# huggingface/distil-whisper

Measured on AMD Instinct MI355X. Metric: training audio-seconds/s (distil-large-v3 student, 30 s clips), higher is better.
Workload: dtype bf16

## Files before the change

distil_whisper_amd/csrc/attention.hip:

```cpp
#include "common.h"
#include "../../include/dwamd.h"

#define NEG_BIG (-1.0e30f)
#ifndef DW_ATTN_DEFER
#define DW_ATTN_DEFER 8
#endif
typedef __attribute__((ext_vector_type(4))) unsigned u32x4;

struct AttnP {
    const bf16* q; const bf16* k; const bf16* v; bf16* o; float* lse;
    const bf16* d_o; float* delta; bf16* dq; bf16* dk; bf16* dv;
    long ldq, ldk, ldv, ldo, lddo, lddq, lddk, lddv;
    int B, H, Lq, Lk;
    long q_rows, kv_rows;
    float* dq_colsum;
    float* dv_colsum;
    const int* q_start; const int* q_len;
    const int* kv_start; const int* kv_len;
    int kv_B;
    int plain_order;
    float defer;
    int coff;
    float scale;
};

__device__ __forceinline__ bf16x8 pack8(const f32x16& x, int s2) {
    bf16x8 r;
#pragma unroll
    for (int e = 0; e < 8; ++e) r[e] = f2bf(x[s2 * 8 + e]);
    return r;
}

__device__ __forceinline__ bf16x8 ldg8(const bf16* base, long row, long ld, int col) {
    return *(const bf16x8*)(base + row * ld + col);
}

__device__ __forceinline__ void store_t(bf16* base, long ld, long row, bool ok, int cb, int hi, const f32x16& a,
                                        float mul) {
    if (!ok) return;
#pragma unroll
    for (int g = 0; g < 4; ++g) {
        bf16x4 w;
#pragma unroll
        for (int e = 0; e < 4; ++e) w[e] = f2bf(a[g * 4 + e] * mul);
        *(bf16x4*)(base + row * ld + cb * 32 + g * 8 + hi * 4) = w;
    }
}

__device__ __forceinline__ void store_rows(bf16* base, long ld, int row0, int nrows, char* patch, int lane,
                                           const f32x16& a0, const f32x16& a1, float mul) {
    const int hi = lane >> 5, ln = lane & 31;
    char* const wr = patch + ln * 144 + hi * 8;
#pragma unroll
    for (int cb = 0; cb < 2; ++cb) {
        const f32x16& a = cb == 0 ? a0 : a1;
#pragma unroll
        for (int g = 0; g < 4; ++g) {
            bf16x4 w;
#pragma unroll
            for (int e = 0; e < 4; ++e) w[e] = f2bf(a[g * 4 + e] * mul);
            *(bf16x4*)(wr + cb * 64 + g * 16) = w;
        }
    }
    const int rr = lane >> 3, sc = lane & 7;
    u32x4 o[4];
#pragma unroll
    for (int it = 0; it < 4; ++it) o[it] = *(const u32x4*)(patch + (it * 8 + rr) * 144 + sc * 16);
    const unsigned loff = (unsigned)(rr * (int)ld + sc * 8) * 2u;
    char* const rb = (char*)(base + (long)row0 * ld);
#pragma unroll
    for (int it = 0; it < 4; ++it)
        if (row0 + it * 8 + rr < nrows) *(u32x4*)(rb + (long)it * 8 * ld * 2 + loff) = o[it];
}

__device__ __forceinline__ void colsum_t(float* colsum, bool ok, int cb, int hi, int ln, const f32x16& a, float mul) {
#pragma unroll
    for (int r = 0; r < 16; ++r) {
        float v = ok ? bf2f(f2bf(a[r] * mul)) : 0.f;
#pragma unroll
        for (int o = 1; o < 32; o <<= 1) v += __shfl_xor(v, o);
        if (ln == 0) atomicAdd(colsum + cb * 32 + (r & 3) + 8 * (r >> 2) + 4 * hi, v);
    }
}

__device__ __forceinline__ void attn_workgroup(int ntile, int H, bool plain, int& tile, int& h, int& b) {
    const int n = gridDim.x, L = blockIdx.x;
    const int xcd = L & 7, slot = L >> 3, q = n >> 3, r = n & 7;
    const int logical = plain ? L : xcd * q + min(xcd, r) + slot;
    tile = logical % ntile;
    const int bh = logical / ntile;
    h = bh % H;
    b = bh / H;
}

template <bool CAUSAL, bool VL = false>
__global__ __launch_bounds__(256, CAUSAL ? 2 : 4) void attn_fwd_kernel(const AttnP p) {
    constexpr int NW = 4;
    __shared__ __attribute__((aligned(1024))) char smem[2 * 16384];
    const int lane = threadIdx.x & 63;
    const int wave = __builtin_amdgcn_readfirstlane(threadIdx.x >> 6);
    const int hi = lane >> 5, ln = lane & 31;
    int tile, h, b;
    attn_workgroup((p.Lq + 32 * NW - 1) / (32 * NW), p.H, p.plain_order, tile, h, b);
    const int qb0 = tile * (32 * NW);
    long q_row0 = (long)b * p.q_rows, kv_row0 = (long)b * p.kv_rows;
    int Lq = p.Lq, Lk = p.Lk;
    if constexpr (VL) {
        q_row0 = p.q_start[b];
        Lq = p.q_len[b];
        if (p.kv_start) { kv_row0 = p.kv_start[b]; Lk = p.kv_len[b]; }
        else kv_row0 = (long)min(b, p.kv_B - 1) * p.kv_rows;
        if (qb0 >= Lq) return;
    }
    const int q = qb0 + wave * 32 + ln;
    const bool q_ok = q < Lq;
    const int qc = q_ok ? q : Lq - 1;
    const bf16* Q = p.q + q_row0 * p.ldq + h * 64;
    const bf16* K = p.k + kv_row0 * p.ldk + h * 64;
    const bf16* V = p.v + kv_row0 * p.ldv + h * 64;

    bf16x8 qf[4];
// ... 156 lines not shown
            const float pb = round_bf16(pv);
            const bf16x8 v8 = *(const bf16x8*)(V + (long)k * p.ldv);
#pragma unroll
            for (int e = 0; e < 8; ++e) o[e] = fmaf(pb, bf2f(v8[e]), o[e]);
        }
    }
    l = (lane & 7) == 0 ? l : 0.f;
    l = wave_sum(l);
#pragma unroll
    for (int e = 0; e < 8; ++e) {
        o[e] += __shfl_xor(o[e], 8);
        o[e] += __shfl_xor(o[e], 16);
        o[e] += __shfl_xor(o[e], 32);
    }
    if (sub == 0) {
#pragma unroll
        for (int e = 0; e < 8; ++e) part[wave * 64 + ds + e] = o[e];
    }
    if (lane == 0) redl[wave] = l;
    __syncthreads();
    if (wave == 0) {
        float acc = 0.f, lt = 0.f;
#pragma unroll
        for (int i = 0; i < NW; ++i) { acc += part[i * 64 + lane]; lt += redl[i]; }
        bf16* O = p.o + (long)b * p.q_rows * p.ldo + h * 64;
        O[lane] = f2bf(acc / lt);
        if (p.lse && lane == 0) p.lse[(long)b * p.H + h] = (mx + __log2f(lt)) * 0.6931471805599453f;
    }
}

template <bool CAUSAL>
__global__ __launch_bounds__(256, 3) void attn_bwd_dq_kernel(const AttnP p) {
    constexpr int NW = 4;
    __shared__ __attribute__((aligned(1024))) char smem[2 * 16384];
    const int lane = threadIdx.x & 63;
    const int wave = __builtin_amdgcn_readfirstlane(threadIdx.x >> 6);
    const int hi = lane >> 5, ln = lane & 31;
    int tile, h, b;
    attn_workgroup((p.Lq + 32 * NW - 1) / (32 * NW), p.H, p.plain_order, tile, h, b);
    const int qb0 = tile * (32 * NW);
    const int q = qb0 + wave * 32 + ln;
    const bool q_ok = q < p.Lq;
    const int qc = q_ok ? q : p.Lq - 1;
    const bf16* Q = p.q + (long)b * p.Lq * p.ldq + h * 64;
    const bf16* DO = p.d_o + (long)b * p.Lq * p.lddo + h * 64;
    const bf16* K = p.k + (long)b * p.Lk * p.ldk + h * 64;
    const bf16* V = p.v + (long)b * p.Lk * p.ldv + h * 64;

    bf16x8 qf[4], gf[4];
#pragma unroll
    for (int kk = 0; kk < 4; ++kk) {
        qf[kk] = ldg8(Q, qc, p.ldq, kk * 16 + hi * 8);
        gf[kk] = ldg8(DO, qc, p.lddo, kk * 16 + hi * 8);
    }
    const long sidx = ((long)b * p.H + h) * p.Lq + qc;
    const float c = p.scale * 1.4426950408889634f;
    float dsum = 0.f;
    {
        const bf16* Orow = p.o + (long)b * p.Lq * p.ldo + h * 64;
#pragma unroll
        for (int kk = 0; kk < 4; ++kk) {
            const bf16x8 o8 = ldg8(Orow, qc, p.ldo, kk * 16 + hi * 8);
#pragma unroll
            for (int e = 0; e < 8; ++e) dsum += bf2f(o8[e]) * bf2f(gf[kk][e]);
        }
        dsum = xhalf_sum(dsum);
    }
// ... 55 lines not shown
                        const int key = kt * 64 + kb * 32 + ((r + e) & 3) + 8 * ((r + e) >> 2) + 4 * hi_o;
                        pv[e] = (key < p.Lk && (!CAUSAL || key <= q_o)) ? pv[e] : 0.f;
                    }
                }
                const f32x2 d2 = {dp[r], dp[r + 1]};
                pv = pv * d2;
                s[r] = pv[0];
                s[r + 1] = pv[1];
            }
#pragma unroll
            for (int s2 = 0; s2 < 2; ++s2) {
                const bf16x8 df = pack8(s, s2);
                const int rb = kb * 32 + s2 * 16 + hi * 4;
#pragma unroll
                for (int db = 0; db < 2; ++db)
                    acc[db] = __builtin_amdgcn_mfma_f32_32x32x16_bf16(frag_tr(tK, db, rb, rb + 8, lane), df, acc[db], 0, 0, 0);
            }
        }
    }
    };
    if constexpr (CAUSAL) tiles(std::integral_constant<int, 2>{}, 0, nkt);
    else {
        const int nfull = p.Lk >> 6;
        tiles(std::integral_constant<int, 0>{}, 0, nfull);
        tiles(std::integral_constant<int, 1>{}, nfull, nkt);
    }
    bf16* DQ = p.dq + (long)b * p.Lq * p.lddq + h * 64;
    if ((p.lddq & 7) == 0 && ((uintptr_t)p.dq & 15) == 0) {
        __syncthreads();
        store_rows(DQ, p.lddq, qb0 + wave * 32, p.Lq, smem + wave * 4608, lane, acc[0], acc[1], p.scale);
    } else {
        store_t(DQ, p.lddq, q, q_ok, 0, hi, acc[0], p.scale);
        store_t(DQ, p.lddq, q, q_ok, 1, hi, acc[1], p.scale);
    }
    if (p.dq_colsum) {
        colsum_t(p.dq_colsum + ((long)b * p.H + h) * 64, q_ok, 0, hi, ln, acc[0], p.scale);
        colsum_t(p.dq_colsum + ((long)b * p.H + h) * 64, q_ok, 1, hi, ln, acc[1], p.scale);
    }
}

template <bool CAUSAL>
__global__ __launch_bounds__(256, CAUSAL ? 2 : 3) void attn_bwd_dkv_kernel(const AttnP p) {
    constexpr int NW = 4;
    constexpr int STG = 16384 + 512;
    __shared__ __attribute__((aligned(1024))) char smem[2 * 17408];
    const int lane = threadIdx.x & 63;
    const int wave = __builtin_amdgcn_readfirstlane(threadIdx.x >> 6);
    const int hi = lane >> 5, ln = lane & 31;
    int tile, h, b;
    attn_workgroup((p.Lk + 32 * NW - 1) / (32 * NW), p.H, p.plain_order, tile, h, b);
    const int kb0 = tile * (32 * NW);
    const int key = kb0 + wave * 32 + ln;
    const bool k_ok = key < p.Lk;
    const int kc = k_ok ? key : p.Lk - 1;
    const bf16* Q = p.q + (long)b * p.Lq * p.ldq + h * 64;
    const bf16* DO = p.d_o + (long)b * p.Lq * p.lddo + h * 64;
    const bf16* K = p.k + (long)b * p.Lk * p.ldk + h * 64;
    const bf16* V = p.v + (long)b * p.Lk * p.ldv + h * 64;
    const float* DEL = p.delta + ((long)b * p.H + h) * p.Lq;
    const float* LSE = DEL + (long)p.B * p.H * p.Lq;

    bf16x8 kf[4], vf[4];
#pragma unroll
    for (int kk = 0; kk < 4; ++kk) {
        kf[kk] = ldg8(K, kc, p.ldk, kk * 16 + hi * 8);
        vf[kk] = ldg8(V, kc, p.ldv, kk * 16 + hi * 8);
    }
    const float c = p.scale * 1.4426950408889634f;
    const int nqt = (p.Lq + 63) >> 6;
    int qt0 = 0;
    if (CAUSAL) qt0 = kb0 >> 6;
    f32x16 av[2], ak[2];
#pragma unroll
    for (int r = 0; r < 16; ++r) { av[0][r] = 0.f; av[1][r] = 0.f; ak[0][r] = 0.f; ak[1][r] = 0.f; }

    auto stage = [&](int qt, int buf, int lane) __attribute__((always_inline)) {
        char* base = smem + buf * 17408;
        stage_tile64<NW>(Q, p.ldq, qt * 64, p.Lq, base, wave, lane);
// ... 67 lines not shown
                s[r + 1] = pv[1];
            }
#pragma unroll
            for (int s2 = 0; s2 < 2; ++s2) {
                const bf16x8 pf = pack8(pr, s2);
                const bf16x8 df = pack8(s, s2);
                const int rb = qb * 32 + s2 * 16 + hi * 4;
#pragma unroll
                for (int db = 0; db < 2; ++db) {
                    av[db] = __builtin_amdgcn_mfma_f32_32x32x16_bf16(frag_tr(tG, db, rb, rb + 8, lane), pf, av[db], 0, 0, 0);
                    ak[db] = __builtin_amdgcn_mfma_f32_32x32x16_bf16(frag_tr(tQ, db, rb, rb + 8, lane), df, ak[db], 0, 0, 0);
                }
            }
        }
    }
    };
    if constexpr (CAUSAL) tiles(std::integral_constant<int, 2>{}, qt0, nqt);
    else {
        const int nfull = kb0 + 32 * NW - 1 >= p.Lk ? 0 : (p.Lq >> 6);
        tiles(std::integral_constant<int, 0>{}, 0, nfull);
        tiles(std::integral_constant<int, 1>{}, nfull, nqt);
    }
    bf16* DK = p.dk + (long)b * p.Lk * p.lddk + h * 64;
    bf16* DV = p.dv + (long)b * p.Lk * p.lddv + h * 64;
    if (((p.lddk | p.lddv) & 7) == 0 && (((uintptr_t)p.dk | (uintptr_t)p.dv) & 15) == 0) {
        __syncthreads();
        store_rows(DK, p.lddk, kb0 + wave * 32, p.Lk, smem + wave * 4608, lane, ak[0], ak[1], p.scale);
        store_rows(DV, p.lddv, kb0 + wave * 32, p.Lk, smem + wave * 4608, lane, av[0], av[1], 1.0f);
    } else {
        store_t(DK, p.lddk, key, k_ok, 0, hi, ak[0], p.scale);
        store_t(DK, p.lddk, key, k_ok, 1, hi, ak[1], p.scale);
        store_t(DV, p.lddv, key, k_ok, 0, hi, av[0], 1.0f);
        store_t(DV, p.lddv, key, k_ok, 1, hi, av[1], 1.0f);
    }
    if (p.dv_colsum) {
        colsum_t(p.dv_colsum + ((long)b * p.H + h) * 64, k_ok, 0, hi, ln, av[0], 1.0f);
        colsum_t(p.dv_colsum + ((long)b * p.H + h) * 64, k_ok, 1, hi, ln, av[1], 1.0f);
    }
}

int g_attn_plain_order = 0;
int g_attn_defer = DW_ATTN_DEFER;
int g_attn_decode = 1;
static int check_ld(int64_t ld) { return (ld & 7) ? DW_EINVAL : DW_OK; }

extern "C" int dw_attn_fwd_ex(const void* q, const void* k, const void* v, void* o, float* lse, int B, int H, int Lq,
                              int Lk, int64_t ldq, int64_t ldk, int64_t ldv, int64_t ldo, int64_t q_batch_rows,
                              int64_t kv_batch_rows, int causal, float scale, void* stream);

extern "C" int dw_attn_fwd(const void* q, const void* k, const void* v, void* o, float* lse, int B, int H, int Lq,
                           int Lk, int64_t ldq, int64_t ldk, int64_t ldv, int64_t ldo, int causal, float scale,
                           void* stream) {
    if (!lse) return DW_EINVAL;
    return dw_attn_fwd_ex(q, k, v, o, lse, B, H, Lq, Lk, ldq, ldk, ldv, ldo, Lq, Lk, causal, scale, stream);
}

extern "C" int dw_attn_fwd_ex(const void* q, const void* k, const void* v, void* o, float* lse, int B, int H, int Lq,
                              int Lk, int64_t ldq, int64_t ldk, int64_t ldv, int64_t ldo, int64_t q_batch_rows,
                              int64_t kv_batch_rows, int causal, float scale, void* stream) {
    DW_CLEAR_ERR();
    if (!q || !k || !v || !o || B <= 0 || H <= 0 || Lq <= 0 || Lk <= 0) return DW_EINVAL;
    if (q_batch_rows < Lq || kv_batch_rows < Lk) return DW_EINVAL;
    if ((int64_t)Lk * ldk >= (1LL << 31) || (int64_t)Lk * ldv >= (1LL << 31)) return DW_EINVAL;
    if (check_ld(ldq) || check_ld(ldk) || check_ld(ldv) || (ldo & 3)) return DW_EINVAL;
    if (((uintptr_t)q & 15) || ((uintptr_t)k & 15) || ((uintptr_t)v & 15) || ((uintptr_t)o & 7)) return DW_EINVAL;
    AttnP p = {};
    p.q = (const bf16*)q; p.k = (const bf16*)k; p.v = (const bf16*)v; p.o = (bf16*)o; p.lse = lse;
    p.ldq = ldq; p.ldk = ldk; p.ldv = ldv; p.ldo = ldo;
    p.B = B; p.H = H; p.Lq = Lq; p.Lk = Lk; p.scale = scale;
    p.q_rows = q_batch_rows; p.kv_rows = kv_batch_rows;
    if (causal != 0 && causal != 1 && causal != 2) return DW_EINVAL;
// ... 28 lines not shown
    if (check_ld(ldq) || check_ld(ldk) || check_ld(ldv) || (ldo & 7)) return DW_EINVAL;
    if (((uintptr_t)q & 15) || ((uintptr_t)k & 15) || ((uintptr_t)v & 15) || ((uintptr_t)o & 15)) return DW_EINVAL;
    const int64_t lk_max = kv_start ? max_q : Lk;
    if (lk_max * ldk >= (1LL << 31) || lk_max * ldv >= (1LL << 31)) return DW_EINVAL;
    AttnP p = {};
    p.q = (const bf16*)q; p.k = (const bf16*)k; p.v = (const bf16*)v; p.o = (bf16*)o; p.lse = nullptr;
    p.ldq = ldq; p.ldk = ldk; p.ldv = ldv; p.ldo = ldo;
    p.B = n_seq; p.H = H; p.Lq = max_q; p.Lk = kv_start ? max_q : Lk; p.scale = scale;
    p.q_rows = 0; p.kv_rows = kv_batch_rows; p.coff = 0;
    p.q_start = q_start; p.q_len = q_len; p.kv_start = kv_start; p.kv_len = kv_len; p.kv_B = kv_batches;
    p.plain_order = g_attn_plain_order;
    p.defer = (float)g_attn_defer;
    hipStream_t s = (hipStream_t)stream;
    dim3 grid(((max_q + 127) / 128) * H * n_seq), block(256);
    if (causal) hipLaunchKernelGGL((attn_fwd_kernel<true, true>), grid, block, 0, s, p);
    else hipLaunchKernelGGL((attn_fwd_kernel<false, true>), grid, block, 0, s, p);
    DW_CHECK_LAUNCH();
    return DW_OK;
}

extern "C" int dw_attn_bwd_ex(const void* q, const void* k, const void* v, const void* o, const void* d_o,
                              const float* lse, float* delta, void* dq, void* dk, void* dv, int B, int H, int Lq, int Lk,
                              int64_t ldq, int64_t ldk, int64_t ldv, int64_t ldo, int64_t lddo, int64_t lddq,
                              int64_t lddk, int64_t lddv, int causal, float scale, float* dq_colsum, float* dv_colsum,
                              void* stream);
extern "C" int dw_attn_bwd(const void* q, const void* k, const void* v, const void* o, const void* d_o,
                           const float* lse, float* delta, void* dq, void* dk, void* dv, int B, int H, int Lq, int Lk,
                           int64_t ldq, int64_t ldk, int64_t ldv, int64_t ldo, int64_t lddo, int64_t lddq,
                           int64_t lddk, int64_t lddv, int causal, float scale, void* stream) {
    return dw_attn_bwd_ex(q, k, v, o, d_o, lse, delta, dq, dk, dv, B, H, Lq, Lk, ldq, ldk, ldv, ldo, lddo, lddq, lddk, lddv,
                          causal, scale, nullptr, nullptr, stream);
}

extern "C" int dw_attn_bwd_ex(const void* q, const void* k, const void* v, const void* o, const void* d_o,
                              const float* lse, float* delta, void* dq, void* dk, void* dv, int B, int H, int Lq, int Lk,
                              int64_t ldq, int64_t ldk, int64_t ldv, int64_t ldo, int64_t lddo, int64_t lddq,
                              int64_t lddk, int64_t lddv, int causal, float scale, float* dq_colsum, float* dv_colsum,
                              void* stream) {
    DW_CLEAR_ERR();
    if (!q || !k || !v || !o || !d_o || !lse || !delta || !dq || !dk || !dv) return DW_EINVAL;
    if (B <= 0 || H <= 0 || Lq <= 0 || Lk <= 0) return DW_EINVAL;
    if (causal != 0 && causal != 1) return DW_EINVAL;
    if (check_ld(ldq) || check_ld(ldk) || check_ld(ldv) || check_ld(ldo) || check_ld(lddo)) return DW_EINVAL;
    if ((lddq & 3) || (lddk & 3) || (lddv & 3)) return DW_EINVAL;
    if ((int64_t)Lk * ldk >= (1LL << 31) || (int64_t)Lk * ldv >= (1LL << 31) || (int64_t)Lq * ldq >= (1LL << 31) ||
        (int64_t)Lq * lddo >= (1LL << 31))
        return DW_EINVAL;
    if (((uintptr_t)q & 15) || ((uintptr_t)k & 15) || ((uintptr_t)v & 15) || ((uintptr_t)o & 15) ||
        ((uintptr_t)d_o & 15) || ((uintptr_t)dq & 7) || ((uintptr_t)dk & 7) || ((uintptr_t)dv & 7))
        return DW_EINVAL;
    AttnP p = {};
    p.q = (const bf16*)q; p.k = (const bf16*)k; p.v = (const bf16*)v; p.o = (bf16*)o; p.lse = (float*)lse;
    p.d_o = (const bf16*)d_o; p.delta = delta; p.dq = (bf16*)dq; p.dk = (bf16*)dk; p.dv = (bf16*)dv;
    p.ldq = ldq; p.ldk = ldk; p.ldv = ldv; p.ldo = ldo; p.lddo = lddo; p.lddq = lddq; p.lddk = lddk; p.lddv = lddv;
    p.B = B; p.H = H; p.Lq = Lq; p.Lk = Lk; p.scale = scale;
    p.dq_colsum = dq_colsum; p.dv_colsum = dv_colsum;
    hipStream_t s = (hipStream_t)stream;
    dim3 gq(((Lq + 127) / 128) * H * B), gk(((Lk + 127) / 128) * H * B), block(256);
    p.plain_order = g_attn_plain_order;
    p.defer = (float)g_attn_defer;
    if (causal) hipLaunchKernelGGL(attn_bwd_dq_kernel<true>, gq, block, 0, s, p);
    else hipLaunchKernelGGL(attn_bwd_dq_kernel<false>, gq, block, 0, s, p);
    if (causal) hipLaunchKernelGGL(attn_bwd_dkv_kernel<true>, gk, block, 0, s, p);
    else hipLaunchKernelGGL(attn_bwd_dkv_kernel<false>, gk, block, 0, s, p);
    DW_CHECK_LAUNCH();
    return DW_OK;
}
```

distil_whisper_amd/csrc/elementwise.hip:

```cpp
#include "common.h"
#include "../../include/dwamd.h"

template <bool TBF, bool OBF>
__global__ __launch_bounds__(256) void embed_fwd_kernel(const int64_t* ids, const void* tok, const void* pos, void* out,
                                                        int T, int D, long nvec) {
    const long i = (long)blockIdx.x * 256 + threadIdx.x;
    if (i >= nvec) return;
    const int dv = D >> 2;
    const long row = i / dv;
    const int c = (int)(i - row * dv) * 4;
    const int t = (int)(row % T);
    const long id = ids[row];
    f32x4 a, b;
    if (TBF) {
        const bf16x4 x = *(const bf16x4*)((const bf16*)tok + id * D + c);
        const bf16x4 y = *(const bf16x4*)((const bf16*)pos + (long)t * D + c);
#pragma unroll
        for (int e = 0; e < 4; ++e) { a[e] = bf2f(x[e]); b[e] = bf2f(y[e]); }
    } else {
        a = *(const f32x4*)((const float*)tok + id * D + c);
        b = *(const f32x4*)((const float*)pos + (long)t * D + c);
    }
    if (OBF) {
        bf16x4 o;
// ... 345 lines not shown
}

extern "C" int dw_cast_f32_bf16(const float* x, void* y, int64_t n, void* stream) {
    DW_CLEAR_ERR();
    if (!x || !y || n <= 0 || ((uintptr_t)x & 15) || ((uintptr_t)y & 7)) return DW_EINVAL;
    hipLaunchKernelGGL(cast_f32_bf16_kernel, dim3(((n + 3) / 4 + 255) / 256), dim3(256), 0, (hipStream_t)stream, x,
                       (bf16*)y, (long)n);
    DW_CHECK_LAUNCH();
    return DW_OK;
}
extern "C" int dw_cast_bf16_f32(const void* x, float* y, int64_t n, void* stream) {
    DW_CLEAR_ERR();
    if (!x || !y || n <= 0 || ((uintptr_t)x & 7) || ((uintptr_t)y & 15)) return DW_EINVAL;
    hipLaunchKernelGGL(cast_bf16_f32_kernel, dim3(((n + 3) / 4 + 255) / 256), dim3(256), 0, (hipStream_t)stream,
                       (const bf16*)x, y, (long)n);
    DW_CHECK_LAUNCH();
    return DW_OK;
}

extern "C" int dw_colsum_bf16(const void* x, int64_t ld, int rows, int cols, float* out, int accumulate,
                              void* stream) {
    DW_CLEAR_ERR();
    if (!x || !out || rows <= 0 || cols <= 0 || (cols & 7) || (ld & 7) || ((uintptr_t)x & 15)) return DW_EINVAL;
    hipStream_t s = (hipStream_t)stream;
    if (!accumulate) hipLaunchKernelGGL(zero_f32_kernel, dim3((cols + 255) / 256), dim3(256), 0, s, out, cols);
    int ry = (rows + 15) / 16;
    if (ry > 64) ry = 64;
    hipLaunchKernelGGL(colsum_kernel, dim3((cols + 127) / 128, ry), dim3(256), 0, s, (const bf16*)x, (long)ld, rows,
                       cols, out);
    DW_CHECK_LAUNCH();
    return DW_OK;
}

extern "C" int dw_add(const void* a, int a_dtype, const void* b, int b_dtype, void* y, int y_dtype, int64_t n,
                      void* stream) {
    DW_CLEAR_ERR();
    if (!a || !b || !y || n <= 0) return DW_EINVAL;
    long nb = (n + 255) / 256;
    if (nb > 4096) nb = 4096;
    hipLaunchKernelGGL(add_kernel, dim3(nb), dim3(256), 0, (hipStream_t)stream, a, a_dtype, b, b_dtype, y, y_dtype,
                       (long)n);
    DW_CHECK_LAUNCH();
    return DW_OK;
}

extern "C" int dw_move_rows(const void* src, int64_t src_pitch_bytes, void* dst, int64_t dst_pitch_bytes,
                            const int32_t* idx, int n, int row_bytes, int scatter, void* stream) {
    DW_CLEAR_ERR();
    if (!src || !dst || !idx || n <= 0 || row_bytes <= 0 || (row_bytes & 15) || (src_pitch_bytes & 15) ||
        (dst_pitch_bytes & 15) || ((uintptr_t)src & 15) || ((uintptr_t)dst & 15))
        return DW_EINVAL;
    const int vpr = row_bytes >> 4;
    const long nv = (long)n * vpr;
    hipLaunchKernelGGL(move_rows_kernel, dim3((nv + 255) / 256), dim3(256), 0, (hipStream_t)stream, (const char*)src,
                       (long)src_pitch_bytes, (char*)dst, (long)dst_pitch_bytes, idx, n, vpr, scatter);
    DW_CHECK_LAUNCH();
    return DW_OK;
}

extern "C" int dw_selftest_tr16(int32_t* out, void* stream) {
    DW_CLEAR_ERR();
    if (!out) return DW_EINVAL;
    hipLaunchKernelGGL(selftest_tr16_kernel, dim3(1), dim3(64), 0, (hipStream_t)stream, out);
    DW_CHECK_LAUNCH();
    return DW_OK;
}
// ... 1 lines not shown
```

distil_whisper_amd/ops_hip.py:

```python
import ctypes as C
import math
import os

import torch

from .decoding import SEQUENCE_BIAS_MAX_SEQUENCES, SEQUENCE_BIAS_MAX_TOKENS

_HERE = os.path.dirname(os.path.abspath(__file__))
LIB_PATH = os.path.join(_HERE, "libdwamd.so")

DW_F32, DW_BF16 = 0, 1


class DwGemm(C.Structure):
    _fields_ = [
        ("a", C.c_void_p), ("b", C.c_void_p), ("c", C.c_void_p), ("bias", C.c_void_p), ("z_out", C.c_void_p),
        ("zgrad_in", C.c_void_p), ("r", C.c_void_p),
        ("lda", C.c_int64), ("ldb", C.c_int64), ("ldc", C.c_int64), ("ldz", C.c_int64), ("ldzg", C.c_int64),
        ("ldr", C.c_int64),
        ("m", C.c_int32), ("n", C.c_int32), ("k", C.c_int32),
        ("trans_a", C.c_int32), ("trans_b", C.c_int32), ("act", C.c_int32), ("c_dtype", C.c_int32),
        ("r_dtype", C.c_int32), ("r_row_mod", C.c_int32), ("round_res", C.c_int32), ("tile", C.c_int32),
        ("split_k", C.c_int32), ("atomic_acc", C.c_int32), ("slice_stride", C.c_int64),
        ("ln_x", C.c_void_p), ("ln_gamma", C.c_void_p), ("ln_beta", C.c_void_p), ("kv_out", C.c_void_p),
# ... 27 lines not shown
                             C.c_float, C.c_void_p], C.c_int),
    "dw_decode_attn_proj_rows": ([C.c_void_p, C.c_int, C.c_int64, C.c_void_p, C.c_void_p, C.c_float, C.c_void_p, C.c_void_p, C.c_void_p,
                                  C.c_void_p, C.c_int64, C.c_int64, C.c_void_p, C.c_void_p, C.c_int64, C.c_int, C.c_int, C.c_float,
                                  C.c_void_p, C.c_int32, C.c_void_p], C.c_int),
    "dw_decode_token_rows": ([C.POINTER(DwDecodeStep), C.c_void_p, C.c_int32, C.c_void_p], C.c_int),
    "dw_cross_kv_quant": ([C.c_void_p, C.c_int64, C.c_void_p, C.c_void_p, C.c_void_p, C.c_int, C.c_int, C.c_int, C.c_int, C.c_void_p],
                          C.c_int),
    "dw_decode_attn_proj_kv8": ([C.c_void_p, C.c_int, C.c_int64, C.c_void_p, C.c_void_p, C.c_float, C.c_void_p, C.c_void_p, C.c_void_p,
                                 C.c_void_p, C.c_void_p, C.c_int64, C.c_void_p, C.c_int64, C.c_int, C.c_int, C.c_int, C.c_float,
                                 C.c_void_p], C.c_int),
    "dw_slot_step": ([C.c_void_p, C.c_int, C.c_int, C.c_int64, C.c_void_p, C.c_void_p] + [C.c_int] * 4 + [C.c_void_p, C.c_int64] +
                     [C.c_void_p] * 7, C.c_int),
    "dw_slot_step_scores": ([C.c_void_p, C.c_int, C.c_int, C.c_int64, C.c_void_p, C.c_void_p] + [C.c_int] * 4 +
                            [C.c_void_p, C.c_int64] + [C.c_void_p] * 9 + [C.c_int, C.c_void_p], C.c_int),
    "dw_logmel": ([C.c_void_p, C.c_int, C.c_int, C.c_void_p, C.c_int, C.c_void_p, C.c_void_p, C.c_void_p, C.c_void_p,
                   C.c_void_p], C.c_int),
    "dw_gemm_bf16": ([C.POINTER(DwGemm), C.c_void_p], C.c_int),
    "dw_layernorm_fwd": ([C.c_void_p, C.c_int, C.c_void_p, C.c_void_p, C.c_void_p, C.c_void_p, C.c_void_p, C.c_int,
                          C.c_int, C.c_float, C.c_void_p], C.c_int),
    "dw_layernorm_bwd": ([C.c_void_p, C.c_void_p, C.c_int, C.c_void_p, C.c_void_p, C.c_void_p, C.c_void_p, C.c_int,
                          C.c_void_p, C.c_void_p, C.c_void_p, C.c_void_p, C.c_int, C.c_int, C.c_void_p, C.c_int64, C.c_void_p], C.c_int),
    "dw_layernorm_bwd_ws_bytes": ([C.c_int, C.c_int], C.c_int),
    "dw_reduce_slices_ld": ([C.c_void_p, C.c_int64, C.c_int64, C.c_int, C.c_void_p, C.c_int64, C.c_int, C.c_int, C.c_int, C.c_void_p], C.c_int),
    "dw_layernorm_fwd_ld": ([C.c_void_p, C.c_int, C.c_void_p, C.c_void_p, C.c_void_p, C.c_void_p, C.c_void_p, C.c_int,
                             C.c_int, C.c_float, C.c_int64, C.c_int64, C.c_void_p], C.c_int),
    "dw_layernorm_bwd_ld": ([C.c_void_p, C.c_void_p, C.c_int, C.c_void_p, C.c_void_p, C.c_void_p, C.c_void_p, C.c_int,
                             C.c_void_p, C.c_void_p, C.c_void_p, C.c_void_p, C.c_int, C.c_int] + [C.c_int64] * 4 + [C.c_void_p, C.c_int64, C.c_void_p], C.c_int),
    "dw_attn_fwd": ([C.c_void_p] * 5 + [C.c_int] * 4 + [C.c_int64] * 4 + [C.c_int, C.c_float, C.c_void_p], C.c_int),
    "dw_attn_fwd_ex": ([C.c_void_p] * 5 + [C.c_int] * 4 + [C.c_int64] * 6 + [C.c_int, C.c_float, C.c_void_p], C.c_int),
    "dw_attn_fwd_varlen": ([C.c_void_p] * 4 + [C.c_int] * 4 + [C.c_int64] * 4 + [C.c_void_p] * 4 + [C.c_int, C.c_int64, C.c_int, C.c_float,
                                                                                                           C.c_void_p], C.c_int),
    "dw_attn_bwd": ([C.c_void_p] * 10 + [C.c_int] * 4 + [C.c_int64] * 8 + [C.c_int, C.c_float, C.c_void_p], C.c_int),
    "dw_attn_bwd_ex": ([C.c_void_p] * 10 + [C.c_int] * 4 + [C.c_int64] * 8 + [C.c_int, C.c_float] + [C.c_void_p] * 3, C.c_int),
    "dw_distill_loss": ([C.c_void_p, C.c_void_p, C.c_void_p, C.c_int, C.c_int, C.c_int64, C.c_float, C.c_float,
                         C.c_float, C.c_float, C.c_void_p, C.c_void_p, C.c_void_p, C.c_void_p, C.c_void_p,
                         C.c_void_p], C.c_int),
    "dw_distill_loss_w": ([C.c_void_p, C.c_void_p, C.c_void_p, C.c_int, C.c_int, C.c_int64, C.c_float, C.c_void_p,
                           C.c_float, C.c_void_p, C.c_void_p, C.c_void_p, C.c_void_p, C.c_void_p, C.c_void_p], C.c_int),
    "dw_embed_fwd": ([C.c_void_p, C.c_void_p, C.c_void_p, C.c_int, C.c_void_p, C.c_int, C.c_int, C.c_int, C.c_int,
                      C.c_void_p], C.c_int),
    "dw_embed_bwd": ([C.c_void_p, C.c_void_p, C.c_void_p, C.c_void_p, C.c_int, C.c_int, C.c_int, C.c_void_p], C.c_int),
    "dw_im2col_mel": ([C.c_void_p, C.c_void_p, C.c_int, C.c_int, C.c_int, C.c_int, C.c_void_p], C.c_int),
    "dw_im2col_s2": ([C.c_void_p, C.c_void_p, C.c_int, C.c_int, C.c_int, C.c_void_p], C.c_int),
    "dw_col2im_s2_gelu_bwd": ([C.c_void_p, C.c_void_p, C.c_void_p, C.c_int, C.c_int, C.c_int, C.c_void_p], C.c_int),
    "dw_gelu_bwd": ([C.c_void_p, C.c_int, C.c_void_p, C.c_void_p, C.c_int64, C.c_void_p], C.c_int),
    "dw_pack_conv_weight": ([C.c_void_p, C.c_void_p, C.c_int, C.c_int, C.c_int, C.c_void_p], C.c_int),
    "dw_unpack_conv_grad": ([C.c_void_p, C.c_void_p, C.c_int, C.c_int, C.c_int, C.c_int, C.c_void_p], C.c_int),
    "dw_cast_f32_bf16": ([C.c_void_p, C.c_void_p, C.c_int64, C.c_void_p], C.c_int),
    "dw_cast_bf16_f32": ([C.c_void_p, C.c_void_p, C.c_int64, C.c_void_p], C.c_int),
    "dw_colsum_bf16": ([C.c_void_p, C.c_int64, C.c_int, C.c_int, C.c_void_p, C.c_int, C.c_void_p], C.c_int),
    "dw_add": ([C.c_void_p, C.c_int, C.c_void_p, C.c_int, C.c_void_p, C.c_int, C.c_int64, C.c_void_p], C.c_int),
    "dw_move_rows": ([C.c_void_p, C.c_int64, C.c_void_p, C.c_int64, C.c_void_p, C.c_int, C.c_int, C.c_int, C.c_void_p], C.c_int),
    "dw_sumsq_f32": ([C.c_void_p, C.c_int64, C.c_void_p, C.c_void_p, C.c_void_p], C.c_int),
    "dw_adamw": ([C.c_void_p] * 5 + [C.c_int64, C.c_void_p] + [C.c_float] * 2 + [C.c_double] * 5 + [C.c_int, C.c_void_p], C.c_int),
    "dw_adam_tick": ([C.c_void_p, C.c_void_p, C.c_void_p], C.c_int),
    "dw_adamw_dev": ([C.c_void_p] * 5 + [C.c_int64, C.c_void_p] + [C.c_float] * 2 + [C.c_void_p] + [C.c_double] * 2 +
                     [C.c_void_p], C.c_int),
    "dw_selftest_tr16": ([C.c_void_p, C.c_void_p], C.c_int),
    "dw_debug_set": ([C.c_int, C.c_int], C.c_int),
    "dw_reduce_slices": ([C.c_void_p, C.c_int64, C.c_int, C.c_void_p, C.c_int64, C.c_int, C.c_void_p], C.c_int),
    "dw_greedy_select": ([C.c_void_p, C.c_int, C.c_int, C.c_int64, C.c_void_p, C.c_void_p] + [C.c_int] * 5 +
                         [C.c_void_p, C.c_int64, C.c_int, C.c_int, C.c_int, C.c_int, C.c_void_p, C.c_void_p,
                          C.c_void_p], C.c_int),
    "dw_greedy_select_history": ([C.c_void_p, C.c_int, C.c_int, C.c_int64, C.c_void_p, C.c_void_p] + [C.c_int] * 5 +
                                 [C.c_void_p, C.c_int64, C.c_int, C.c_int, C.c_int, C.c_int, C.c_void_p, C.c_void_p,
                                  C.c_float, C.c_int, C.c_void_p], C.c_int),
# ... 375 lines not shown
                                              v.stride(0), out.stride(0), _p(q_start), _p(q_len),
                                              _p(q_start) if self_attention else None, _p(q_len) if self_attention else None,
                                              int(kv_batches), int(Lk), int(causal), float(scale), self._stream()), "attn_fwd_varlen")
        self._t1(e0, "attn_fwd", flops)
        return out

    def attn_fwd(self, q, k, v, B, H, Lq, Lk, causal, scale, out=None, kv_batch_rows=None):
        for t in (q, k, v):
            assert t.dtype == torch.bfloat16 and t.stride(1) == 1
        o = self.empty((B * Lq, H * 64), torch.bfloat16) if out is None else out
        assert o.dtype == torch.bfloat16 and o.stride(1) == 1 and o.shape == (B * Lq, H * 64)
        lse = self.empty((B, H, Lq), torch.float32)
        e0 = self._t0()
        self._chk(self.lib.dw_attn_fwd_ex(_p(q), _p(k), _p(v), _p(o), _p(lse), B, H, Lq, Lk, q.stride(0), k.stride(0),
                                          v.stride(0), o.stride(0), Lq, Lk if kv_batch_rows is None else kv_batch_rows,
                                          int(causal), float(scale), self._stream()), "attn_fwd")
        self._t1(e0, "attn_fwd", 4.0 * B * H * Lq * Lk * 64)
        return o, lse

    def attn_bwd(self, q, k, v, o, do, lse, B, H, Lq, Lk, causal, scale, dq=None, dk=None, dv=None, dq_colsum=None,
                 dv_colsum=None):
        if dq is None:
            dq = self.empty((B * Lq, H * 64), torch.bfloat16)
        if dk is None:
            dk = self.empty((B * Lk, H * 64), torch.bfloat16)
        if dv is None:
            dv = self.empty((B * Lk, H * 64), torch.bfloat16)
        delta = self.empty((2, B, H, Lq), torch.float32)
        for t in (q, k, v, o, do, dq, dk, dv):
            assert t.dtype == torch.bfloat16 and t.stride(1) == 1
        e0 = self._t0()
        for t in (dq_colsum, dv_colsum):
            assert t is None or (t.dtype == torch.float32 and t.numel() == H * 64 and t.is_contiguous())
        part = None
        if dq_colsum is not None or dv_colsum is not None:
            key = (B, H)
            if not hasattr(self, "_attn_cs"):
                self._attn_cs = {}
            if key not in self._attn_cs:
                self._attn_cs[key] = self.zeros((2, B, H * 64), torch.float32)
            part = self._attn_cs[key]
            part.zero_()
        self._chk(self.lib.dw_attn_bwd_ex(_p(q), _p(k), _p(v), _p(o), _p(do), _p(lse), _p(delta), _p(dq), _p(dk), _p(dv),
                                          B, H, Lq, Lk, q.stride(0), k.stride(0), v.stride(0), o.stride(0), do.stride(0),
                                          dq.stride(0), dk.stride(0), dv.stride(0), int(causal), float(scale),
                                          _p(part[0]) if dq_colsum is not None else None,
                                          _p(part[1]) if dv_colsum is not None else None, self._stream()), "attn_bwd")
        for i, dst in enumerate((dq_colsum, dv_colsum)):
            if dst is not None:
                self._chk(self.lib.dw_reduce_slices(_p(part[i]), H * 64, B, _p(dst), H * 64, 1, self._stream()),
                          "reduce_slices")
        self._t1(e0, "attn_bwd", 10.0 * B * H * Lq * Lk * 64)
        return dq, dk, dv

    def distill_loss(self, s_logits, t_logits, labels, V, temperature, ce_weight, kl_weight, grad_scale, want_grad,
                     grad_out=None, weights_dev=None, return_rows=False):
        rows, ld = s_logits.shape
        if grad_out is not None:
            assert want_grad and grad_out.shape == s_logits.shape and grad_out.dtype == torch.bfloat16 and grad_out.is_contiguous()
        assert s_logits.dtype == torch.bfloat16 and t_logits.dtype == torch.bfloat16
        assert s_logits.is_contiguous() and t_logits.is_contiguous() and t_logits.shape == s_logits.shape
        assert labels.dtype == torch.int64 and labels.numel() == rows and labels.is_contiguous()
        losses = self.empty((4,), torch.float32)
        row_ce = self.empty((rows,), torch.float32)
        row_kl = self.empty((rows,), torch.float32)
        counts = self.empty((2,), torch.int32)
        dl = (_p(s_logits) if grad_out is None else _p(grad_out)) if want_grad else None
        if weights_dev is not None:
            assert weights_dev.dtype == torch.float32 and weights_dev.numel() == 2 and weights_dev.is_contiguous()
            self._chk(self.lib.dw_distill_loss_w(_p(s_logits), _p(t_logits), _p(labels), rows, V, ld, float(temperature),
                                                 _p(weights_dev), float(grad_scale), _p(losses), dl, _p(row_ce), _p(row_kl),
                                                 _p(counts), self._stream()), "distill_loss_w")
            return (losses, row_ce, row_kl) if return_rows else losses
        self._chk(self.lib.dw_distill_loss(_p(s_logits), _p(t_logits), _p(labels), rows, V, ld, float(temperature),
                                           float(ce_weight), float(kl_weight), float(grad_scale), _p(losses), dl,
                                           _p(row_ce), _p(row_kl), _p(counts),
                                           self._stream()), "distill_loss")
        return (losses, row_ce, row_kl) if return_rows else losses

    def embed_fwd(self, ids, tok, pos, out_dtype, rows_alloc=0, out=None):
        B, T = ids.shape
        D = tok.shape[1]
        assert ids.dtype == torch.int64 and ids.is_contiguous() and tok.is_contiguous() and pos.is_contiguous()
        assert tok.dtype == pos.dtype
# ... 430 lines not shown
```

include/dwamd.h:

```cpp
#ifndef DWAMD_H
#define DWAMD_H
#include <stdint.h>
#ifdef __cplusplus
extern "C" {
#endif

#define DW_OK 0
#define DW_EINVAL (-1)
#define DW_EUNSUP (-2)

#define DW_F32 0
#define DW_BF16 1

int dw_version(void);

int dw_logmel(const float* audio, int batch, int n_samples, const float* mel_filters, int n_mels,
              const float* twiddle, const float* window, float* out, float* clipmax, void* stream);

typedef struct DwGemm {
    const void* a;
    const void* b;
    void* c;
    const float* bias;
    void* z_out;
// ... 27 lines not shown
int dw_reduce_slices_ld(const float* part, int64_t slice_stride, int64_t ld_part, int slices, float* out, int64_t ld_out,
                        int rows, int cols, int accumulate, void* stream);

int dw_layernorm_fwd(const void* x, int x_dtype, const float* gamma, const float* beta, void* y, float* mean,
                     float* rstd, int rows, int cols, float eps, void* stream);
int dw_layernorm_bwd_ws_bytes(int rows, int cols);
int dw_layernorm_bwd(const void* dy_bf16, const void* x, int x_dtype, const float* mean, const float* rstd,
                     const float* gamma, float* dres, int accumulate, float* dgamma, float* dbeta, void* dres_lowp,
                     float* dres_colsum, int rows, int cols, void* sums, int64_t sums_bytes, void* stream);
int dw_layernorm_fwd_ld(const void* x, int x_dtype, const float* gamma, const float* beta, void* y, float* mean,
                        float* rstd, int rows, int cols, float eps, int64_t ldx, int64_t ldy, void* stream);
int dw_layernorm_bwd_ld(const void* dy_bf16, const void* x, int x_dtype, const float* mean, const float* rstd,
                        const float* gamma, float* dres, int accumulate, float* dgamma, float* dbeta, void* dres_lowp,
                        float* dres_colsum, int rows, int cols, int64_t lddy, int64_t ldx, int64_t lddres,
                        int64_t ldlowp, void* sums, int64_t sums_bytes, void* stream);

int dw_attn_fwd(const void* q, const void* k, const void* v, void* o, float* lse, int B, int H, int Lq, int Lk,
                int64_t ldq, int64_t ldk, int64_t ldv, int64_t ldo, int causal, float scale, void* stream);
int dw_attn_fwd_ex(const void* q, const void* k, const void* v, void* o, float* lse, int B, int H, int Lq, int Lk,
                   int64_t ldq, int64_t ldk, int64_t ldv, int64_t ldo, int64_t q_batch_rows, int64_t kv_batch_rows,
                   int causal, float scale, void* stream);
int dw_attn_fwd_varlen(const void* q, const void* k, const void* v, void* o, int n_seq, int H, int max_q, int Lk, int64_t ldq,
                       int64_t ldk, int64_t ldv, int64_t ldo, const int32_t* q_start, const int32_t* q_len,
                       const int32_t* kv_start, const int32_t* kv_len, int kv_batches, int64_t kv_batch_rows, int causal,
                       float scale, void* stream);
int dw_attn_bwd(const void* q, const void* k, const void* v, const void* o, const void* d_o, const float* lse,
                float* delta, void* dq, void* dk, void* dv, int B, int H, int Lq, int Lk, int64_t ldq, int64_t ldk,
                int64_t ldv, int64_t ldo, int64_t lddo, int64_t lddq, int64_t lddk, int64_t lddv, int causal,
                float scale, void* stream);
int dw_attn_bwd_ex(const void* q, const void* k, const void* v, const void* o, const void* d_o, const float* lse,
                   float* delta, void* dq, void* dk, void* dv, int B, int H, int Lq, int Lk, int64_t ldq, int64_t ldk,
                   int64_t ldv, int64_t ldo, int64_t lddo, int64_t lddq, int64_t lddk, int64_t lddv, int causal,
                   float scale, float* dq_colsum, float* dv_colsum, void* stream);

int dw_distill_loss(const void* s_logits, const void* t_logits, const int64_t* labels, int rows, int V, int64_t ld,
                    float temperature, float ce_weight, float kl_weight, float grad_scale, float* losses,
                    void* dlogits, float* row_ce, float* row_kl, int32_t* counts, void* stream);
int dw_distill_loss_w(const void* s_logits, const void* t_logits, const int64_t* labels, int rows, int V, int64_t ld,
                      float temperature, const float* weights, float grad_scale, float* losses, void* dlogits,
                      float* row_ce, float* row_kl, int32_t* counts, void* stream);

int dw_embed_fwd(const int64_t* ids, const void* tok, const void* pos, int tab_dtype, void* out, int out_dtype,
                 int B, int T, int D, void* stream);
int dw_embed_bwd(const float* dx, const int64_t* ids, float* dtok, float* dpos, int B, int T, int D, void* stream);

int dw_im2col_mel(const float* mel, void* xcol, int B, int C, int T, int kpad, void* stream);
int dw_im2col_s2(const void* a, void* xcol, int B, int T, int C, void* stream);
int dw_col2im_s2_gelu_bwd(const void* dxcol, const void* z, void* dz, int B, int T, int C, void* stream);
int dw_gelu_bwd(const void* dy, int dy_dtype, const void* z, void* dz, int64_t n, void* stream);
int dw_pack_conv_weight(const float* w, void* wp_bf16, int D, int C, int kpad, void* stream);
int dw_unpack_conv_grad(const float* gwp, float* gw, int D, int C, int kpad, int accumulate, void* stream);

int dw_cast_f32_bf16(const float* x, void* y, int64_t n, void* stream);
int dw_cast_bf16_f32(const void* x, float* y, int64_t n, void* stream);
int dw_colsum_bf16(const void* x, int64_t ld, int rows, int cols, float* out, int accumulate, void* stream);
int dw_move_rows(const void* src, int64_t src_pitch_bytes, void* dst, int64_t dst_pitch_bytes, const int32_t* idx, int n,
                 int row_bytes, int scatter, void* stream);
int dw_add(const void* a, int a_dtype, const void* b, int b_dtype, void* y, int y_dtype, int64_t n, void* stream);

#define DW_SUMSQ_PARTIALS 2048
int dw_sumsq_f32(const float* g, int64_t n, float* out, float* partials, void* stream);
int dw_adamw(float* p, const float* g, float* m, float* v, void* shadow_bf16, int64_t n, const float* sumsq,
             float max_norm, float grad_mul, double lr, double beta1, double beta2, double eps, double weight_decay,
             int step, void* stream);
int dw_adam_tick(double* state, const float* gate, void* stream);
int dw_adamw_dev(float* p, const float* g, float* m, float* v, void* shadow_bf16, int64_t n, const float* sumsq,
// ... 135 lines not shown
```

Baseline: 2887.

## Replace atomic column-sum bias reduction with per-block partials and fold kernel

The attention backward previously built the dq/dv bias gradients by shuffle-reducing every row and issuing global atomicAdds into a per-batch buffer, which then needed a zero fill and a reduce_slices launch. Now each workgroup reuses the LDS patch (or fills it) to sum its 128 rows deterministically and writes one 64-wide partial per tile. A small fold kernel then sums the partials over batch and tiles in double precision and adds the result into the bias gradient. This removes atomic contention and the zeroing, at the cost of an extra __syncthreads, slightly more LDS per block, and a workspace allocation on each call.

```diff
diff --git a/distil_whisper_amd/csrc/attention.hip b/distil_whisper_amd/csrc/attention.hip
--- a/distil_whisper_amd/csrc/attention.hip
+++ b/distil_whisper_amd/csrc/attention.hip
@@ -15,6 +15,8 @@
     long q_rows, kv_rows;
     float* dq_colsum;
     float* dv_colsum;
+    float* dq_part;
+    float* dv_part;
     const int* q_start; const int* q_len;
     const int* kv_start; const int* kv_len;
     int kv_B;
@@ -47,21 +49,24 @@
     }
 }
 
+__device__ __forceinline__ void patch_fill(char* patch, int lane, const f32x16& a0, const f32x16& a1, float mul) {
+    const int hi = lane >> 5, ln = lane & 31;
+    char* const wr = patch + ln * 144 + hi * 8;
+#pragma unroll
+    for (int cb = 0; cb < 2; ++cb) {
+        const f32x16& a = cb == 0 ? a0 : a1;
+#pragma unroll
+        for (int g = 0; g < 4; ++g) {
+            bf16x4 w;
+#pragma unroll
+            for (int e = 0; e < 4; ++e) w[e] = f2bf(a[g * 4 + e] * mul);
+            *(bf16x4*)(wr + cb * 64 + g * 16) = w;
+        }
+    }
+}
 __device__ __forceinline__ void store_rows(bf16* base, long ld, int row0, int nrows, char* patch, int lane,
                                            const f32x16& a0, const f32x16& a1, float mul) {
-    const int hi = lane >> 5, ln = lane & 31;
-    char* const wr = patch + ln * 144 + hi * 8;
-#pragma unroll
-    for (int cb = 0; cb < 2; ++cb) {
-        const f32x16& a = cb == 0 ? a0 : a1;
-#pragma unroll
-        for (int g = 0; g < 4; ++g) {
-            bf16x4 w;
-#pragma unroll
-            for (int e = 0; e < 4; ++e) w[e] = f2bf(a[g * 4 + e] * mul);
-            *(bf16x4*)(wr + cb * 64 + g * 16) = w;
-        }
-    }
+    patch_fill(patch, lane, a0, a1, mul);
     const int rr = lane >> 3, sc = lane & 7;
     u32x4 o[4];
 #pragma unroll
@@ -83,10 +88,30 @@
     }
 }
 
-__device__ __forceinline__ void attn_workgroup(int ntile, int H, bool plain, int& tile, int& h, int& b) {
+typedef __attribute__((address_space(3))) const bf16 lds_cbf16_t;
+typedef __attribute__((address_space(3))) float lds_f32_t;
+__device__ __forceinline__ void colsum_block(float* slot, unsigned red_lds, unsigned patch_lds, int row0, int nrows, int wave, int lane) {
+    const int n = nrows - row0;
+    lds_f32_t* const red = (lds_f32_t*)red_lds;
+    float s = 0.f;
+#pragma unroll
+    for (int r = 0; r < 32; ++r) {
+        const float v = bf2f(*(lds_cbf16_t*)(patch_lds + r * 144 + lane * 2));
+        s += r < n ? v : 0.f;
+    }
+    red[wave * 64 + lane] = s;
+    __syncthreads();
+    const int t = wave * 64 + lane;
+    if (t < 64) slot[t] = ((red[t] + red[64 + t]) + red[128 + t]) + red[192 + t];
+}
+
+__device__ __forceinline__ int attn_logical(bool plain) {
     const int n = gridDim.x, L = blockIdx.x;
     const int xcd = L & 7, slot = L >> 3, q = n >> 3, r = n & 7;
-    const int logical = plain ? L : xcd * q + min(xcd, r) + slot;
+    return plain ? L : xcd * q + min(xcd, r) + slot;
+}
+__device__ __forceinline__ void attn_workgroup(int ntile, int H, bool plain, int& tile, int& h, int& b) {
+    const int logical = attn_logical(plain);
     tile = logical % ntile;
     const int bh = logical / ntile;
     h = bh % H;
@@ -309,7 +334,8 @@
 template <bool CAUSAL>
 __global__ __launch_bounds__(256, 3) void attn_bwd_dq_kernel(const AttnP p) {
     constexpr int NW = 4;
-    __shared__ __attribute__((aligned(1024))) char smem[2 * 16384];
+    __shared__ __attribute__((aligned(1024))) char smem[2 * 16384 + 256 * NW];
+    float* const red = (float*)(smem + 2 * 16384);
     const int lane = threadIdx.x & 63;
     const int wave = __builtin_amdgcn_readfirstlane(threadIdx.x >> 6);
     const int hi = lane >> 5, ln = lane & 31;
@@ -431,18 +457,26 @@
     } else {
         store_t(DQ, p.lddq, q, q_ok, 0, hi, acc[0], p.scale);
         store_t(DQ, p.lddq, q, q_ok, 1, hi, acc[1], p.scale);
+        if (p.dq_part) {
+            __syncthreads();
+            patch_fill(smem + wave * 4608, lane, acc[0], acc[1], p.scale);
+        }
     }
     if (p.dq_colsum) {
         colsum_t(p.dq_colsum + ((long)b * p.H + h) * 64, q_ok, 0, hi, ln, acc[0], p.scale);
         colsum_t(p.dq_colsum + ((long)b * p.H + h) * 64, q_ok, 1, hi, ln, acc[1], p.scale);
     }
+    if (p.dq_part)
+        colsum_block(p.dq_part + (long)attn_logical(p.plain_order) * 64, lds_addr_of(red), lds_addr_of(smem + wave * 4608),
+                     qb0 + wave * 32, p.Lq, wave, lane);
 }
 
 template <bool CAUSAL>
 __global__ __launch_bounds__(256, CAUSAL ? 2 : 3) void attn_bwd_dkv_kernel(const AttnP p) {
     constexpr int NW = 4;
     constexpr int STG = 16384 + 512;
-    __shared__ __attribute__((aligned(1024))) char smem[2 * 17408];
+    __shared__ __attribute__((aligned(1024))) char smem[2 * 17408 + 256 * NW];
+    float* const red = (float*)(smem + 2 * 17408);
     const int lane = threadIdx.x & 63;
     const int wave = __builtin_amdgcn_readfirstlane(threadIdx.x >> 6);
     const int hi = lane >> 5, ln = lane & 31;
@@ -576,11 +610,18 @@
         store_t(DK, p.lddk, key, k_ok, 1, hi, ak[1], p.scale);
         store_t(DV, p.lddv, key, k_ok, 0, hi, av[0], 1.0f);
         store_t(DV, p.lddv, key, k_ok, 1, hi, av[1], 1.0f);
+        if (p.dv_part) {
+            __syncthreads();
+            patch_fill(smem + wave * 4608, lane, av[0], av[1], 1.0f);
+        }
     }
     if (p.dv_colsum) {
         colsum_t(p.dv_colsum + ((long)b * p.H + h) * 64, k_ok, 0, hi, ln, av[0], 1.0f);
         colsum_t(p.dv_colsum + ((long)b * p.H + h) * 64, k_ok, 1, hi, ln, av[1], 1.0f);
     }
+    if (p.dv_part)
+        colsum_block(p.dv_part + (long)attn_logical(p.plain_order) * 64, lds_addr_of(red), lds_addr_of(smem + wave * 4608),
+                     kb0 + wave * 32, p.Lk, wave, lane);
 }
 
 int g_attn_plain_order = 0;
@@ -675,11 +716,54 @@
                           causal, scale, nullptr, nullptr, stream);
 }
 
+int attn_bias_fold(const float* pq, int ntq, float* oq, const float* pv, int ntk, float* ov, int B, int H, hipStream_t s);
+
+static int attn_bwd_launch(const void* q, const void* k, const void* v, const void* o, const void* d_o,
+                           const float* lse, float* delta, void* dq, void* dk, void* dv, int B, int H, int Lq, int Lk,
+                           int64_t ldq, int64_t ldk, int64_t ldv, int64_t ldo, int64_t lddo, int64_t lddq,
+                           int64_t lddk, int64_t lddv, int causal, float scale, float* dq_colsum, float* dv_colsum,
+                           float* dq_part, float* dv_part, void* stream);
+
 extern "C" int dw_attn_bwd_ex(const void* q, const void* k, const void* v, const void* o, const void* d_o,
                               const float* lse, float* delta, void* dq, void* dk, void* dv, int B, int H, int Lq, int Lk,
                               int64_t ldq, int64_t ldk, int64_t ldv, int64_t ldo, int64_t lddo, int64_t lddq,
                               int64_t lddk, int64_t lddv, int causal, float scale, float* dq_colsum, float* dv_colsum,
                               void* stream) {
+    return attn_bwd_launch(q, k, v, o, d_o, lse, delta, dq, dk, dv, B, H, Lq, Lk, ldq, ldk, ldv, ldo, lddo, lddq, lddk, lddv,
+                           causal, scale, dq_colsum, dv_colsum, nullptr, nullptr, stream);
+}
+
+static int64_t attn_bias_slots(int B, int H, int L) { return (int64_t)B * H * ((L + 127) / 128) * 64; }
+
+extern "C" int dw_attn_bwd_bias_ws_bytes(int B, int H, int Lq, int Lk) {
+    if (B <= 0 || H <= 0 || Lq <= 0 || Lk <= 0) return 0;
+    const int64_t n = (attn_bias_slots(B, H, Lq) + attn_bias_slots(B, H, Lk)) * 4;
+    return n < (1LL << 31) ? (int)n : 0;
+}
+
+extern "C" int dw_attn_bwd_bias(const void* q, const void* k, const void* v, const void* o, const void* d_o,
+                                const float* lse, float* delta, void* dq, void* dk, void* dv, int B, int H, int Lq, int Lk,
+                                int64_t ldq, int64_t ldk, int64_t ldv, int64_t ldo, int64_t lddo, int64_t lddq,
+                                int64_t lddk, int64_t lddv, int causal, float scale, float* dq_bias, float* dv_bias,
+                                void* ws, int64_t ws_bytes, void* stream) {
+    if (!dq_bias && !dv_bias)
+        return attn_bwd_launch(q, k, v, o, d_o, lse, delta, dq, dk, dv, B, H, Lq, Lk, ldq, ldk, ldv, ldo, lddo, lddq, lddk, lddv,
+                               causal, scale, nullptr, nullptr, nullptr, nullptr, stream);
+    const int need = dw_attn_bwd_bias_ws_bytes(B, H, Lq, Lk);
+    if (!ws || need <= 0 || ws_bytes < need || ((uintptr_t)ws & 3)) return DW_EINVAL;
+    float* pq = dq_bias ? (float*)ws : nullptr;
+    float* pv = dv_bias ? (float*)ws + attn_bias_slots(B, H, Lq) : nullptr;
+    const int rc = attn_bwd_launch(q, k, v, o, d_o, lse, delta, dq, dk, dv, B, H, Lq, Lk, ldq, ldk, ldv, ldo, lddo, lddq, lddk,
+                                   lddv, causal, scale, nullptr, nullptr, pq, pv, stream);
+    if (rc != DW_OK) return rc;
+    return attn_bias_fold(pq, (Lq + 127) / 128, dq_bias, pv, (Lk + 127) / 128, dv_bias, B, H, (hipStream_t)stream);
+}
+
+static int attn_bwd_launch(const void* q, const void* k, const void* v, const void* o, const void* d_o,
+                           const float* lse, float* delta, void* dq, void* dk, void* dv, int B, int H, int Lq, int Lk,
+                           int64_t ldq, int64_t ldk, int64_t ldv, int64_t ldo, int64_t lddo, int64_t lddq,
+                           int64_t lddk, int64_t lddv, int causal, float scale, float* dq_colsum, float* dv_colsum,
+                           float* dq_part, float* dv_part, void* stream) {
     DW_CLEAR_ERR();
     if (!q || !k || !v || !o || !d_o || !lse || !delta || !dq || !dk || !dv) return DW_EINVAL;
     if (B <= 0 || H <= 0 || Lq <= 0 || Lk <= 0) return DW_EINVAL;
@@ -698,6 +782,7 @@
     p.ldq = ldq; p.ldk = ldk; p.ldv = ldv; p.ldo = ldo; p.lddo = lddo; p.lddq = lddq; p.lddk = lddk; p.lddv = lddv;
     p.B = B; p.H = H; p.Lq = Lq; p.Lk = Lk; p.scale = scale;
     p.dq_colsum = dq_colsum; p.dv_colsum = dv_colsum;
+    p.dq_part = dq_part; p.dv_part = dv_part;
     hipStream_t s = (hipStream_t)stream;
     dim3 gq(((Lq + 127) / 128) * H * B), gk(((Lk + 127) / 128) * H * B), block(256);
     p.plain_order = g_attn_plain_order;
diff --git a/distil_whisper_amd/csrc/elementwise.hip b/distil_whisper_amd/csrc/elementwise.hip
--- a/distil_whisper_amd/csrc/elementwise.hip
+++ b/distil_whisper_amd/csrc/elementwise.hip
@@ -401,6 +401,35 @@
     return DW_OK;
 }
 
+__global__ __launch_bounds__(512) void attn_bias_fold_kernel(const float* pq, int ntq, float* oq, const float* pv, int ntk, float* ov,
+                                                             int B, int H) {
+    __shared__ double sh[8][64];
+    const float* part = blockIdx.y ? pv : pq;
+    float* out = blockIdx.y ? ov : oq;
+    const int nt = blockIdx.y ? ntk : ntq;
+    if (!part) return;
+    const int h = blockIdx.x, c = threadIdx.x & 63, g = threadIdx.x >> 6;
+    double s = 0.0;
+    for (int j = g; j < B * nt; j += 8) {
+        const int b = j / nt, tile = j - b * nt;
+        s += (double)part[(((long)b * H + h) * nt + tile) * 64 + c];
+    }
+    sh[g][c] = s;
+    __syncthreads();
+    if (g == 0) {
+        double t = sh[0][c];
+#pragma unroll
+        for (int i = 1; i < 8; ++i) t += sh[i][c];
+        out[h * 64 + c] += (float)t;
+    }
+}
+
+int attn_bias_fold(const float* pq, int ntq, float* oq, const float* pv, int ntk, float* ov, int B, int H, hipStream_t s) {
+    hipLaunchKernelGGL(attn_bias_fold_kernel, dim3(H, 2), dim3(512), 0, s, pq, ntq, oq, pv, ntk, ov, B, H);
+    DW_CHECK_LAUNCH();
+    return DW_OK;
+}
+
 extern "C" int dw_add(const void* a, int a_dtype, const void* b, int b_dtype, void* y, int y_dtype, int64_t n,
                       void* stream) {
     DW_CLEAR_ERR();
diff --git a/distil_whisper_amd/ops_hip.py b/distil_whisper_amd/ops_hip.py
--- a/distil_whisper_amd/ops_hip.py
+++ b/distil_whisper_amd/ops_hip.py
@@ -83,6 +83,9 @@
                                                                                                            C.c_void_p], C.c_int),
     "dw_attn_bwd": ([C.c_void_p] * 10 + [C.c_int] * 4 + [C.c_int64] * 8 + [C.c_int, C.c_float, C.c_void_p], C.c_int),
     "dw_attn_bwd_ex": ([C.c_void_p] * 10 + [C.c_int] * 4 + [C.c_int64] * 8 + [C.c_int, C.c_float] + [C.c_void_p] * 3, C.c_int),
+    "dw_attn_bwd_bias_ws_bytes": ([C.c_int] * 4, C.c_int),
+    "dw_attn_bwd_bias": ([C.c_void_p] * 10 + [C.c_int] * 4 + [C.c_int64] * 8 + [C.c_int, C.c_float] + [C.c_void_p] * 3 +
+                         [C.c_int64, C.c_void_p], C.c_int),
     "dw_distill_loss": ([C.c_void_p, C.c_void_p, C.c_void_p, C.c_int, C.c_int, C.c_int64, C.c_float, C.c_float,
                          C.c_float, C.c_float, C.c_void_p, C.c_void_p, C.c_void_p, C.c_void_p, C.c_void_p,
                          C.c_void_p], C.c_int),
@@ -524,24 +527,15 @@
         e0 = self._t0()
         for t in (dq_colsum, dv_colsum):
             assert t is None or (t.dtype == torch.float32 and t.numel() == H * 64 and t.is_contiguous())
-        part = None
+        ws, ws_bytes = None, 0
         if dq_colsum is not None or dv_colsum is not None:
-            key = (B, H)
-            if not hasattr(self, "_attn_cs"):
-                self._attn_cs = {}
-            if key not in self._attn_cs:
-                self._attn_cs[key] = self.zeros((2, B, H * 64), torch.float32)
-            part = self._attn_cs[key]
-            part.zero_()
-        self._chk(self.lib.dw_attn_bwd_ex(_p(q), _p(k), _p(v), _p(o), _p(do), _p(lse), _p(delta), _p(dq), _p(dk), _p(dv),
-                                          B, H, Lq, Lk, q.stride(0), k.stride(0), v.stride(0), o.stride(0), do.stride(0),
-                                          dq.stride(0), dk.stride(0), dv.stride(0), int(causal), float(scale),
-                                          _p(part[0]) if dq_colsum is not None else None,
-                                          _p(part[1]) if dv_colsum is not None else None, self._stream()), "attn_bwd")
-        for i, dst in enumerate((dq_colsum, dv_colsum)):
-            if dst is not None:
-                self._chk(self.lib.dw_reduce_slices(_p(part[i]), H * 64, B, _p(dst), H * 64, 1, self._stream()),
-                          "reduce_slices")
+            ws_bytes = self.lib.dw_attn_bwd_bias_ws_bytes(B, H, Lq, Lk)
+            assert ws_bytes > 0
+            ws = self.empty((ws_bytes // 4,), torch.float32)
+        self._chk(self.lib.dw_attn_bwd_bias(_p(q), _p(k), _p(v), _p(o), _p(do), _p(lse), _p(delta), _p(dq), _p(dk), _p(dv),
+                                            B, H, Lq, Lk, q.stride(0), k.stride(0), v.stride(0), o.stride(0), do.stride(0),
+                                            dq.stride(0), dk.stride(0), dv.stride(0), int(causal), float(scale),
+                                            _p(dq_colsum), _p(dv_colsum), _p(ws), ws_bytes, self._stream()), "attn_bwd")
         self._t1(e0, "attn_bwd", 10.0 * B * H * Lq * Lk * 64)
         return dq, dk, dv
 
diff --git a/include/dwamd.h b/include/dwamd.h
--- a/include/dwamd.h
+++ b/include/dwamd.h
@@ -83,6 +83,11 @@
                    float* delta, void* dq, void* dk, void* dv, int B, int H, int Lq, int Lk, int64_t ldq, int64_t ldk,
                    int64_t ldv, int64_t ldo, int64_t lddo, int64_t lddq, int64_t lddk, int64_t lddv, int causal,
                    float scale, float* dq_colsum, float* dv_colsum, void* stream);
+int dw_attn_bwd_bias_ws_bytes(int B, int H, int Lq, int Lk);
+int dw_attn_bwd_bias(const void* q, const void* k, const void* v, const void* o, const void* d_o, const float* lse,
+                     float* delta, void* dq, void* dk, void* dv, int B, int H, int Lq, int Lk, int64_t ldq, int64_t ldk,
+                     int64_t ldv, int64_t ldo, int64_t lddo, int64_t lddq, int64_t lddk, int64_t lddv, int causal,
+                     float scale, float* dq_bias, float* dv_bias, void* ws, int64_t ws_bytes, void* stream);
 
 int dw_distill_loss(const void* s_logits, const void* t_logits, const int64_t* labels, int rows, int V, int64_t ld,
                     float temperature, float ce_weight, float kl_weight, float grad_scale, float* losses,
```

After: 2888, median of 2. No clear change (+0.0%).
